# acdha/trivy

Measured on AMD Instinct MI355X. Metric: secret-scan GB/s (builtin rules) at 1/2/4/8 MI355X; % of HBM peak, higher is better.
Workload: dtype u8

## Files before the change

### trivy_amd/csrc/kernels.hip

```cpp
#include <hip/hip_runtime.h>

#include <algorithm>
#include <map>
#include <cstdlib>
#include <cstring>
#include <memory>
#include <vector>

#include "device.hpp"
#include "internal.hpp"
#include "k1f.hpp"

namespace tsg {

#define HIP_TRY(x)                                                                    \
  do {                                                                                \
    hipError_t e_ = (x);                                                              \
    if (e_ != hipSuccess)                                                             \
      return fail(TSG_ERR_GPU, std::string(#x) + ": " + hipGetErrorString(e_));       \
  } while (0)

constexpr int kStreams = 4;
constexpr int kK1Chains = 2;
constexpr int kK1Unroll = 8;
constexpr int kK1Seg = 8;
constexpr int kK1Lds[3] = {52, 80, 156};
constexpr int kK1BlocksPerCU[3] = {3, 2, 1};
constexpr __host__ __device__ int k1_threads(int ldsk) { return ldsk == 156 ? 1024 : 512; }
constexpr uint32_t kK1RepBytes = 256 * 32 * 4;
constexpr int kBlock = 256;
constexpr int kPad = 256;
constexpr int kItemsBpc = 8;
constexpr uint32_t kStampBlocks = 8;
constexpr int kMaxBack = (int)kMaxBackChunks;

struct DevDFA {
  const uint16_t* tab;
  const uint16_t* acc;
  const uint16_t* acc_state;
  const uint16_t* eot;
  const uint16_t* to_ni;
  const uint8_t* dead;
  const uint64_t* masks;
  const uint8_t* cls;
  const uint32_t* rules;
  uint32_t nc, ns, mw, nmasks, state_acc;
  uint32_t nrules;
  uint32_t inv_nc;
  uint32_t start[4];
  uint32_t o_cls, o_dead, o_accs, o_masks, lds_bytes;
};

struct DevK1 {
  const uint16_t* tab;
  const uint32_t* cls;
  const uint32_t* pcls;
  const uint16_t* accs;
  const uint32_t* masks;
  uint32_t nc, ns, nmasks, mw, kw_words, start, warm, kU, kD;
  uint32_t acc_row;
  uint32_t row_unit;
  uint32_t tab_words;
  uint32_t packed;
  uint32_t lds_class;
  uint32_t rep;
  const uint16_t* kw_len;
  uint32_t kw_maxlen;
};

struct DevCand {
  uint32_t file, rule, end;
};

__device__ __forceinline__ uint32_t ctx_of(uint8_t c) {
  if (c == '\n') return 1;
  if ((c >= '0' && c <= '9') || (c >= 'A' && c <= 'Z') || (c >= 'a' && c <= 'z') || c == '_') return 2;
  return 3;
}

__device__ __forceinline__ uint32_t byte_of(const uint4 v, uint32_t k) {
  const uint32_t w = k < 8 ? (k < 4 ? v.x : v.y) : (k < 12 ? v.z : v.w);
  return (w >> ((k & 3) * 8)) & 0xFF;
}

constexpr uint32_t kCfShift = 14;

__device__ __forceinline__ uint32_t bsearch_file(const uint64_t* __restrict__ off, uint32_t lo, uint32_t hi,
                                                 uint64_t p) {
  while (hi - lo > 1) {
    const uint32_t mid = (lo + hi) >> 1;
    if (off[mid] <= p) lo = mid;
    else hi = mid;
  }
  return lo;
}

__device__ __forceinline__ uint32_t file_of(const uint32_t* __restrict__ cf, const uint64_t* __restrict__ off,
                                            uint32_t nfiles, uint64_t p) {
  const uint64_t k = p >> kCfShift;
  return bsearch_file(off, cf[k], min(nfiles, cf[k + 1] + 1), p);
}

__device__ __forceinline__ void stage16(uint8_t* dst, const void* src, uint32_t nbytes) {
// ... 1642 lines not shown
}

__global__ void __launch_bounds__(kBlock) items_emit_kernel(ItemArgs A, LayoutArgs LA) {
  extern __shared__ __attribute__((aligned(16))) uint8_t smem[];
  const ItemLds T = item_lds_load(A, smem);
  uint32_t* s_count = (uint32_t*)(smem + item_lds_bytes(A));
  uint32_t* s_base = s_count + A.G;
  uint32_t* s_gbase = s_base + A.G;
  uint8_t* s_kind = (uint8_t*)(s_gbase + A.G);
  layout_block(LA, s_kind, s_gbase);
  const uint64_t nt = (uint64_t)min(*A.nev, A.evcap) + A.F, stride = (uint64_t)gridDim.x * blockDim.x;
  const uint64_t t0 = (uint64_t)blockIdx.x * blockDim.x + threadIdx.x;
  for (uint32_t g = threadIdx.x; g < A.G; g += blockDim.x) {
    s_base[g] = s_kind[g] == kGroupList ? s_gbase[g] + A.bcount[(size_t)blockIdx.x * A.G + g] : 0u;
    s_count[g] = 0;
  }
  __syncthreads();
  for (uint64_t t = t0; t < nt; t += stride)
    gen_items(A, T, t, [&](uint32_t f, uint32_t g, uint64_t lo, uint64_t hi) {
      if (s_kind[g] != kGroupList) return;
      const uint32_t n = (uint32_t)(hi - lo + 1);
      uint32_t at = s_base[g] + atomicAdd(&s_count[g], n);
      for (uint64_t c = lo; c <= hi; c++) A.items[at++] = make_uint2(f, (uint32_t)c);
    });
}

struct K2Args {
  const uint8_t* data;
  const uint64_t* off;
  const uint32_t* cf;
  uint64_t total, nchunks;
  uint32_t chunk, ext_cap, nfiles;
  const uint32_t* kw;
  uint32_t kw_words;
  const uint32_t* gmask;
  const uint32_t* galways;
  const uint2* items;
  const uint4* entries;
  const uint32_t* nentries;
  const uint4* dentries;
  const uint32_t* ndentries;
  DevCand* cand;
  uint32_t* cand_count;
  uint32_t cand_cap;
  uint8_t* ovf;
  uint8_t* hascand;
  uint32_t* diag;
  uint32_t* claim;
  uint32_t word_recs;
  unsigned long long* etrace;
  unsigned long long* clk;
};
constexpr int kTraceW = 8;
#ifdef K2_TRACE_CTR
__shared__ unsigned long long* s_ectr;
#define K2_CTR(k, op, v) (s_ectr ? (void)op(&s_ectr[k], (unsigned long long)(v)) : (void)0)
#else
#define K2_CTR(k, op, v) ((void)0)
#endif
#ifdef K2_TRACE_PHASE
__shared__ unsigned long long* s_tph;
#define K2_PHASE(k) (s_tph && threadIdx.x == 0 ? (void)(s_tph[k] = wall_clock64()) : (void)0)
#else
#define K2_PHASE(k) ((void)0)
#endif

__device__ __forceinline__ void emit_cand(const K2Args& A, uint32_t file, uint32_t rule, uint64_t end) {
  const unsigned long long m = __ballot(1);
  const uint32_t lane = threadIdx.x & 63;
  const uint32_t leader = (uint32_t)__builtin_ctzll(m);
  uint32_t base = 0;
  if (lane == leader) {
    base = atomicAdd(A.cand_count, (uint32_t)__popcll(m));
    K2_CTR(1, atomicAdd, __popcll(m));
  }
  base = __shfl(base, (int)leader);
  const uint32_t idx = base + (uint32_t)__popcll(m & ((1ull << lane) - 1));
  if (idx < A.cand_cap && (end < kCandWhole || end == (uint64_t)kCandWhole)) {
    A.cand[idx] = DevCand{file, rule, (uint32_t)end};
  } else {
    A.ovf[file] = 1;
    if (idx < A.cand_cap) A.cand[idx] = DevCand{file, rule, 0};
  }
  A.hascand[file] = 1;
}

struct Lane {
  const DevDFA& d;
  const K2Args& A;
  const uint16_t* s_tab;
  const uint8_t* s_cls;
  const uint16_t* s_accs;
  const uint64_t* s_masks;
  uint32_t file;
  uint64_t fs;
  uint32_t group;

  __device__ __forceinline__ void emit(uint32_t mi, uint64_t pos) {
    const uint64_t* m = (d.state_acc && mi < d.nmasks) ? s_masks + (size_t)mi * d.mw : d.masks + (size_t)mi * d.mw;
    for (uint32_t w = 0; w < d.mw; w++)
      for (uint64_t v = m[w]; v; v &= v - 1)
        emit_cand(A, file, d.rules[w * 64 + __builtin_ctzll(v)], pos - fs);
  }

  __device__ __forceinline__ uint32_t state_of(uint32_t row) const { return __umulhi(row, d.inv_nc); }

  __device__ __forceinline__ uint32_t trans(uint32_t ix) const { return kCandTrans | (group << 16) | ix; }
  __device__ __forceinline__ void accept_word(uint32_t s0, const uint4 v, int lo, int hi, uint64_t wb) {
    if (A.word_recs)
      emit_cand(A, file, kCandTrans | kCandWord | (group << 16) | s0, wb + (uint64_t)lo - fs);
    else
      replay_emit(s0, v, lo, hi, wb);
  }
  __device__ __forceinline__ void put(uint32_t idx, uint32_t rule, uint64_t end) const {
    if (idx < A.cand_cap && end < kCandWhole) {
      A.cand[idx] = DevCand{file, rule, (uint32_t)end};
    } else {
      A.ovf[file] = 1;
      if (idx < A.cand_cap) A.cand[idx] = DevCand{file, rule, 0};
    }
    A.hascand[file] = 1;
  }
  __device__ __forceinline__ void replay_emit(uint32_t s0, const uint4 v, int lo, int hi, uint64_t wb) {
    uint32_t n = 0, r = s0;
#pragma unroll
    for (int k = 0; k < 16; k++) {
      const uint32_t e = s_tab[r + s_cls[byte_of(v, k)]];
      const bool in = k >= lo && k < hi;
      n += (in && (e & 0x8000u)) ? 1u : 0u;
      r = in ? (e & 0x7FFFu) : r;
    }
    if (!n) return;
    uint32_t at = atomicAdd(A.cand_count, n);
    K2_CTR(1, atomicAdd, n);
    r = s0;
#pragma unroll
    for (int k = 0; k < 16; k++) {
      const uint32_t ix = r + s_cls[byte_of(v, k)];
      const uint32_t e = s_tab[ix];
      const bool in = k >= lo && k < hi;
      if (in && (e & 0x8000u)) put(at++, trans(ix), wb + k - fs);
      r = in ? (e & 0x7FFFu) : r;
    }
  }

  __device__ __forceinline__ uint32_t step(uint32_t s, uint32_t byte, uint64_t pos) {
    const uint32_t ix = s + s_cls[byte];
    const uint32_t e = s_tab[ix];
    if (__builtin_expect(e & 0x8000u, 0)) emit_cand(A, file, trans(ix), pos - fs);
    return e & 0x7FFFu;
  }

  __device__ __forceinline__ uint32_t fast(uint32_t s, uint32_t byte) const { return s_tab[s + s_cls[byte]]; }

  __device__ __forceinline__ void replay16(uint32_t s, const uint4, uint64_t p) {
#pragma unroll 1
    for (uint32_t k = 0; k < 16; k++) s = step(s, A.data[p + k], p + k);
  }

  __device__ __forceinline__ uint32_t step16(uint32_t s, const uint4 v, uint64_t p) {
    const uint32_t s0 = s;
    uint32_t any = 0;
#pragma unroll
    for (int k = 0; k < 16; k++) {
      const uint32_t e = fast(s, byte_of(v, k));
      any |= e;
      s = e & 0x7FFFu;
    }
    if (__builtin_expect(any & 0x8000u, 0)) replay16(s0, v, p);
    return s;
  }

  __device__ __forceinline__ void tail(uint32_t s, uint64_t fe, uint64_t b) {
    if (b >= fe) {
      const uint32_t m = d.eot[state_of(s)];
      if (m) emit(m, fe);
      return;
    }
    tail_ni(d.to_ni[state_of(s)], fe, b);
  }
  __device__ __forceinline__ void tail_ni(uint32_t s, uint64_t fe, uint64_t b) {
    const uint8_t* data = A.data;
    const uint8_t* dead = s_cls + (d.o_dead - d.o_cls);
    uint64_t q = b;
    uint64_t w = q & ~15ull;
    uint4 cur = *(const uint4*)(data + w);
    while (q < fe && !(dead[state_of(s)] & 1)) {
      if (q - b >= A.ext_cap || (dead[state_of(s)] & 2)) {
        for (uint32_t k = 0; k < d.nrules; k++) emit_cand(A, file, d.rules[k], kCandWhole);
        return;
      }
      const uint4 nxt = *(const uint4*)(data + w + 16);
      const uint64_t e = min(fe, w + 16);
      const int lo = (int)(q - w), hi = (int)(e - w);
      const uint32_t s0 = s;
      uint32_t any = 0;
#pragma unroll
      for (int k = 0; k < 16; k++) {
        const uint32_t t = s_tab[s + s_cls[byte_of(cur, k)]];
        const bool in = k >= lo && k < hi;
        any |= in ? t : 0u;
        s = in ? (t & 0x7FFFu) : s;
      }
      if (__builtin_expect(any & 0x8000u, 0)) accept_word(s0, cur, lo, hi, w);
      q = e;
      cur = nxt;
      w += 16;
    }
    K2_CTR(2, atomicAdd, q - b);
    K2_CTR(3, atomicMax, q - b);
    if (A.diag) {
      const uint32_t n = (uint32_t)min<uint64_t>(q - b, 0xFFFFFFFFull);
      atomicAdd(&A.diag[0], n);
      atomicMax(&A.diag[1], n);
      if (n > 4096) atomicAdd(&A.diag[2], 1u);
    }
    if (q >= fe && !(dead[state_of(s)] & 1)) {
      const uint32_t m = d.eot[state_of(s)];
      if (m) emit(m, fe);
    }
  }

  template <int NS>
  __device__ void streams(uint64_t fe, uint64_t a, uint32_t C) {
    const uint8_t* data = A.data;
    uint32_t s[NS];
#pragma unroll
    for (int i = 0; i < NS; i++) {
      const uint64_t b0 = a + (uint64_t)i * C;
      s[i] = (b0 == fs) ? d.start[0] : d.start[ctx_of(data[b0 - 1])];
    }
    uint4 cur[NS];
#pragma unroll
    for (int i = 0; i < NS; i++) cur[i] = *(const uint4*)(data + a + (uint64_t)i * C);
    for (uint32_t j = 0; j < C; j += 16) {
      uint4 nxt[NS];
#pragma unroll
      for (int i = 0; i < NS; i++) nxt[i] = *(const uint4*)(data + a + (uint64_t)i * C + j + 16);
      uint32_t s0[NS], any[NS];
#pragma unroll
      for (int i = 0; i < NS; i++) {
        s0[i] = s[i];
        any[i] = 0;
      }
#pragma unroll
      for (int k = 0; k < 16; k++)
#pragma unroll
        for (int i = 0; i < NS; i++) {
          const uint32_t e = fast(s[i], byte_of(cur[i], k));
          any[i] |= e;
          s[i] = e & 0x7FFFu;
        }
#pragma unroll
      for (int i = 0; i < NS; i++)
        if (__builtin_expect(any[i] & 0x8000u, 0)) replay16(s0[i], cur[i], a + (uint64_t)i * C + j);
#pragma unroll
      for (int i = 0; i < NS; i++) cur[i] = nxt[i];
    }
#pragma unroll
    for (int i = 0; i < NS; i++) tail(s[i], fe, a + (uint64_t)(i + 1) * C);
  }

  __device__ void piece(uint64_t fe, uint64_t a, uint64_t se) {
    const uint8_t* data = A.data;
    uint32_t s = (a == fs) ? d.start[0] : d.start[ctx_of(data[a - 1])];
    uint64_t p = a;
    while (p < se && (p & 15)) {
      s = step(s, data[p], p);
      p++;
    }
    if (p + 16 <= se) {
      uint4 cur = *(const uint4*)(data + p);
      while (p + 16 <= se) {
        const uint4 nxt = *(const uint4*)(data + p + 16);
        s = step16(s, cur, p);
        cur = nxt;
        p += 16;
      }
    }
    while (p < se) {
      s = step(s, data[p], p);
      p++;
    }
    tail(s, fe, se);
  }
};

__device__ __forceinline__ void stage_dfa(const DevDFA& d, uint8_t* smem) {
  stage16(smem, d.tab, (d.ns * d.nc + 1) / 2 * 4);
  stage16(smem + d.o_cls, d.cls, 256);
  stage16(smem + d.o_dead, d.dead, d.ns);
  if (d.state_acc) {
    stage16(smem + d.o_accs, d.acc_state, d.ns * 2);
    stage16(smem + d.o_masks, d.masks, d.nmasks * d.mw * 8);
  }
  __syncthreads();
}

struct K2Item {
  uint32_t s, file;
  uint32_t lo, hi;
  uint32_t chunk;
  uint64_t fe;
};

template <bool RICH>
__device__ __forceinline__ void k2_list_pair(const DevDFA& d, const K2Args& A, const uint16_t* s_tab,
                                             const uint8_t* s_cls, const uint16_t* s_accs,
                                             const uint64_t* s_masks, uint32_t g, uint32_t first, uint32_t n);

template <bool RICH>
__device__ __forceinline__ void k2_list_entry(const DevDFA& d, const K2Args& A, const uint16_t* s_tab,
                                              const uint8_t* s_cls, const uint16_t* s_accs,
                                              const uint64_t* s_masks, uint4 en) {
  for (uint32_t r0i = 0; r0i < en.z; r0i += 2 * kK2Block)
    k2_list_pair<RICH>(d, A, s_tab, s_cls, s_accs, s_masks, en.x, en.y + r0i, min(en.z - r0i, (uint32_t)(2 * kK2Block)));
}

template <bool RICH>
__device__ __forceinline__ void k2_list_pair(const DevDFA& d, const K2Args& A, const uint16_t* s_tab,
                                             const uint8_t* s_cls, const uint16_t* s_accs,
                                             const uint64_t* s_masks, uint32_t g, uint32_t first, uint32_t n) {
  const uint32_t C = A.chunk;
  K2Item it[2];
  bool live[2];
#pragma unroll
  for (int i = 0; i < 2; i++) {
    const uint32_t k = threadIdx.x + (uint32_t)i * kK2Block;
    live[i] = k < n;
    const uint2 item = A.items[first + (live[i] ? k : 0)];
    it[i].file = item.x;
    it[i].chunk = item.y;
    const uint64_t base = (uint64_t)item.y * C;
    const uint8_t before = base ? A.data[base - 1] : 0;
    const uint64_t fs = A.off[item.x], fe = A.off[item.x + 1];
    const uint64_t a = max(fs, base);
    it[i].fe = fe;
    it[i].lo = (uint32_t)(a - base);
    it[i].hi = live[i] ? (uint32_t)(min(fe, base + C) - base) : it[i].lo;
    it[i].s = a == fs ? d.start[0] : d.start[ctx_of(before)];
  }
  Lane L{d, A, s_tab, s_cls, s_accs, s_masks, 0, 0, g};
  if (C & 127) {
#pragma unroll
    for (int i = 0; i < 2; i++)
      if (live[i]) {
        const uint64_t base = (uint64_t)it[i].chunk * C;
        L.file = it[i].file;
        L.fs = A.off[it[i].file];
        L.piece(A.off[it[i].file + 1], base + it[i].lo, base + it[i].hi);
      }
    return;
  }
  auto word = [&](K2Item& c, uint32_t o, const uint4 v) __attribute__((always_inline)) {
    const int32_t lo = min(16, max(0, (int32_t)c.lo - (int32_t)o));
    const int32_t hi = min(16, max(0, (int32_t)c.hi - (int32_t)o));
    const uint32_t mask = ((1u << hi) - 1u) & ~((1u << lo) - 1u);
    uint32_t s = c.s, any = 0;
    const uint32_t s0 = s;
#pragma unroll
    for (int k = 0; k < 16; k++) {
      const uint32_t e = s_tab[s + s_cls[byte_of(v, k)]];
      const bool in = (mask >> k) & 1u;
      any |= in ? e : 0u;
      s = in ? (e & 0x7FFFu) : s;
    }
    if (__builtin_expect(any & 0x8000u, 0)) {
      if (A.diag) atomicAdd(&A.diag[3], 1u);
      K2_CTR(0, atomicAdd, 1);
      L.file = c.file;
      L.fs = A.off[c.file];
      L.accept_word(s0, v, lo, hi, (uint64_t)c.chunk * C + o);
    }
    c.s = s;
  };
  auto word2 = [&](uint32_t o, const uint4 v0, const uint4 v1) __attribute__((always_inline)) {
    K2Item& c0 = it[0];
    K2Item& c1 = it[1];
    const int32_t lo0 = min(16, max(0, (int32_t)c0.lo - (int32_t)o)), hi0 = min(16, max(0, (int32_t)c0.hi - (int32_t)o));
    const int32_t lo1 = min(16, max(0, (int32_t)c1.lo - (int32_t)o)), hi1 = min(16, max(0, (int32_t)c1.hi - (int32_t)o));
    const uint32_t m0 = ((1u << hi0) - 1u) & ~((1u << lo0) - 1u), m1 = ((1u << hi1) - 1u) & ~((1u << lo1) - 1u);
    uint32_t s0 = c0.s, s1 = c1.s, any0 = 0, any1 = 0;
    const uint32_t r0 = s0, r1 = s1;
#pragma unroll
    for (int k = 0; k < 16; k++) {
      const uint32_t e0 = s_tab[s0 + s_cls[byte_of(v0, k)]];
      const uint32_t e1 = s_tab[s1 + s_cls[byte_of(v1, k)]];
      const bool in0 = (m0 >> k) & 1u, in1 = (m1 >> k) & 1u;
      any0 |= in0 ? e0 : 0u;
      any1 |= in1 ? e1 : 0u;
      s0 = in0 ? (e0 & 0x7FFFu) : s0;
      s1 = in1 ? (e1 & 0x7FFFu) : s1;
    }
    if (__builtin_expect((any0 | any1) & 0x8000u, 0)) {
      if (any0 & 0x8000u) {
        if (A.diag) atomicAdd(&A.diag[3], 1u);
        K2_CTR(0, atomicAdd, 1);
        L.file = c0.file;
        L.fs = A.off[c0.file];
        L.accept_word(r0, v0, lo0, hi0, (uint64_t)c0.chunk * C + o);
      }
      if (any1 & 0x8000u) {
        if (A.diag) atomicAdd(&A.diag[3], 1u);
        K2_CTR(0, atomicAdd, 1);
        L.file = c1.file;
        L.fs = A.off[c1.file];
        L.accept_word(r1, v1, lo1, hi1, (uint64_t)c1.chunk * C + o);
      }
    }
    c0.s = s0;
    c1.s = s1;
  };
  K2_PHASE(1);
  if (__ballot(live[0]) == 0) return;
  const uint32_t lane = threadIdx.x & 63, q = lane & 3;
  const bool b0 = q & 1, b1 = (q >> 1) & 1;
  uint4 x0[4], y0[4];
  const uint8_t* dq = A.data + 16u * q;
#define K2_LOAD_T(X, Y, J, T)                                                                 \
  X[T] = *(const uint4*)(dq + (uint64_t)__shfl(it[0].chunk, (int)((lane & ~3u) + T)) * C + (J)); \
  Y[T] = *(const uint4*)(dq + (uint64_t)__shfl(it[1].chunk, (int)((lane & ~3u) + T)) * C + (J));
#define K2_LOAD(X, Y, J) \
  K2_LOAD_T(X, Y, J, 0)  \
  K2_LOAD_T(X, Y, J, 1)  \
  K2_LOAD_T(X, Y, J, 2)  \
  K2_LOAD_T(X, Y, J, 3)
#define K2_BLOCK(X, Y, J)                                                       \
  quad_transpose4(X, b0, b1);                                                   \
  quad_transpose4(Y, b0, b1);                                                   \
  _Pragma("unroll") for (int w = 0; w < 4; w++) {                              \
    word(it[0], (uint32_t)(J) + 16u * w, X[w]);                                 \
    word(it[1], (uint32_t)(J) + 16u * w, Y[w]);                                 \
  }
  if constexpr (RICH) {
#define K2_BLOCK2(X, Y, J)                                                      \
  quad_transpose4(X, b0, b1);                                                   \
  quad_transpose4(Y, b0, b1);                                                   \
  _Pragma("unroll") for (int w = 0; w < 4; w++) word2((uint32_t)(J) + 16u * w, X[w], Y[w]);
    uint4 x1[4], y1[4];
    K2_LOAD(x0, y0, 0)
    for (uint32_t j = 0; j < C; j += 128) {
      if (j + 64 < C) {
        K2_LOAD(x1, y1, j + 64)
      }
      K2_BLOCK2(x0, y0, j)
      if (j + 64 >= C) break;
      if (j + 128 < C) {
        K2_LOAD(x0, y0, j + 128)
      }
      K2_BLOCK2(x1, y1, j + 64)
    }
#undef K2_BLOCK2
  } else {
    K2_LOAD(x0, y0, 0)
    for (uint32_t j = 0; j < C; j += 64) {
      K2_BLOCK(x0, y0, j)
      if (j + 64 < C) {
        K2_LOAD(x0, y0, j + 64)
      }
    }
  }
#undef K2_LOAD_T
#undef K2_LOAD
#undef K2_BLOCK
  K2_PHASE(2);
  uint32_t ni[2];
#pragma unroll
  for (int i = 0; i < 2; i++) {
    const uint64_t b = (uint64_t)it[i].chunk * C + it[i].hi;
    ni[i] = live[i] && b < it[i].fe ? d.to_ni[L.state_of(it[i].s)] : 0u;
  }
#pragma unroll
  for (int i = 0; i < 2; i++)
    if (live[i]) {
      const uint64_t b = (uint64_t)it[i].chunk * C + it[i].hi;
      L.file = it[i].file;
      L.fs = A.off[it[i].file];
      if (b < it[i].fe)
        L.tail_ni(ni[i], it[i].fe, b);
      else
        L.tail(it[i].s, it[i].fe, b);
    }
  K2_PHASE(3);
}

__device__ __forceinline__ void k2_dense_entry(const DevDFA& d, const K2Args& A, uint32_t g, const uint16_t* s_tab,
                                               const uint8_t* s_cls, const uint16_t* s_accs,
                                               const uint64_t* s_masks, uint4 en) {
  Lane L{d, A, s_tab, s_cls, s_accs, s_masks, 0, 0, g};
  const uint32_t* gm = A.gmask + (size_t)g * A.kw_words;
  const uint32_t always = A.galways[g];
  const uint64_t c0 = en.y + (uint64_t)threadIdx.x * kStreams;
  if (c0 >= (uint64_t)en.y + en.z) return;
  uint64_t a = c0 * A.chunk;
  const uint64_t b = min((c0 + kStreams) * A.chunk, A.total);
  uint32_t f = file_of(A.cf, A.off, A.nfiles, a);
  {
    const uint64_t fs = A.off[f], fe = A.off[f + 1];
    if (b == a + (uint64_t)kStreams * A.chunk && a >= fs && b <= fe) {
      if (group_gated(A.kw + (size_t)f * A.kw_words, gm, A.kw_words, always)) {
        L.file = f;
        L.fs = fs;
        L.template streams<kStreams>(fe, a, A.chunk);
      }
      return;
    }
  }
  while (a < b) {
    const uint64_t fs = A.off[f], fe = A.off[f + 1];
    if (fe <= a) {
      f++;
      continue;
    }
    const uint64_t se = min(b, fe);
    if (group_gated(A.kw + (size_t)f * A.kw_words, gm, A.kw_words, always)) {
      L.file = f;
      L.fs = fs;
      L.piece(fe, a, se);
    }
    a = se;
    f++;
  }
}

template <bool DENSE, bool RICH = false>
__device__ __forceinline__ void k2_run(const DevDFA* __restrict__ dfas, const K2Args& A, const uint4* entries,
                                       uint32_t E, uint32_t* claim, uint8_t* smem) {
  __shared__ uint32_t s_e;
  uint32_t staged = 0xFFFFFFFFu;
  uint32_t prev = 0xFFFFFFFFu;
#ifdef K2_TRACE_CTR
  if (threadIdx.x == 0) s_ectr = nullptr;
#endif
#ifdef K2_TRACE_PHASE
  if (threadIdx.x == 0) s_tph = nullptr;
#endif
  if (E == 0) return;
  bool ran = false;
  for (;;) {
    if (threadIdx.x == 0) s_e = atomicAdd(claim, 1u);
    __syncthreads();
    const uint32_t e = s_e;
    __syncthreads();
    if (!DENSE && A.etrace && threadIdx.x == 0) {
      const unsigned long long now = wall_clock64();
      if (prev != 0xFFFFFFFFu) A.etrace[(size_t)prev * kTraceW + 1] = now;
      if (e < E) {
        const uint4 en = entries[e];
        A.etrace[(size_t)e * kTraceW + 0] = now;
        A.etrace[(size_t)e * kTraceW + 2] = ((unsigned long long)en.x << 32) | en.z;
        A.etrace[(size_t)e * kTraceW + 3] = ((unsigned long long)__builtin_amdgcn_s_getreg(20 | (15 << 11)) << 32) |
                                            (uint32_t)__builtin_amdgcn_s_getreg(4 | (31 << 11));
#ifdef K2_TRACE_CTR
        s_ectr = A.etrace + (size_t)e * kTraceW + 4;
#endif
#ifdef K2_TRACE_PHASE
        s_tph = A.etrace + (size_t)e * kTraceW + 4;
#endif
      }
    }
#if defined(K2_TRACE_CTR) || defined(K2_TRACE_PHASE)
    __syncthreads();
#endif
    prev = e;
    if (e >= E) {
      if (ran && threadIdx.x == 0) atomicMax(&A.clk[kClkK2End], (unsigned long long)wall_clock64());
      break;
    }
    ran = true;
    const uint4 en = entries[e];
    const uint32_t g = __builtin_amdgcn_readfirstlane(en.x);
    const DevDFA& d = dfas[g];
    if (g != staged) {
      stage_dfa(d, smem);
      staged = g;
    }
    K2_PHASE(0);
    const uint16_t* s_tab = (const uint16_t*)smem;
    if (DENSE)
      k2_dense_entry(d, A, g, s_tab, smem + d.o_cls, (const uint16_t*)(smem + d.o_accs), (const uint64_t*)(smem + d.o_masks), en);
    else
      k2_list_entry<RICH>(d, A, s_tab, smem + d.o_cls, (const uint16_t*)(smem + d.o_accs), (const uint64_t*)(smem + d.o_masks), en);
  }
}

__global__ void __launch_bounds__(kK2Block) k2_kernel(const DevDFA* __restrict__ dfas, K2Args A) {
  extern __shared__ __attribute__((aligned(16))) uint8_t smem[];
  k2_run<false>(dfas, A, A.entries, *A.nentries, A.claim, smem);
}
__global__ void __launch_bounds__(kK2Block) __attribute__((amdgpu_waves_per_eu(1, 2)))
k2_kernel_rich(const DevDFA* __restrict__ dfas, K2Args A) {
  extern __shared__ __attribute__((aligned(16))) uint8_t smem[];
  k2_run<false, true>(dfas, A, A.entries, *A.nentries, A.claim, smem);
}

__global__ void __launch_bounds__(kBlock) k2_dense_kernel(const DevDFA* __restrict__ dfas, K2Args A) {
  extern __shared__ __attribute__((aligned(16))) uint8_t smem[];
  k2_run<true>(dfas, A, A.dentries, *A.ndentries, A.claim + 1, smem);
}

template <class T>
static int upload_vec(const std::vector<T>& v, const T** dst, std::vector<void*>* allocs) {
  void* p = nullptr;
  const size_t bytes = (std::max<size_t>(v.size() * sizeof(T), 16) + 15) & ~(size_t)15;
  HIP_TRY(hipMalloc(&p, bytes));
  HIP_TRY(hipMemset(p, 0, bytes));
  if (!v.empty()) HIP_TRY(hipMemcpy(p, v.data(), v.size() * sizeof(T), hipMemcpyHostToDevice));
  allocs->push_back(p);
  *dst = (const T*)p;
  return TSG_OK;
}

static uint32_t align16(uint32_t x) { return (x + 15) & ~15u; }

static int make_device_dfa(const DFA& dd, const std::vector<uint32_t>& rules, DevDFA* out,
                           std::vector<void*>* allocs) {
  if (dd.nstates >= 0x8000) return fail(TSG_ERR_INTERNAL, "DFA too large for u16 tables");
  out->nrules = (uint32_t)rules.size();
  DFA padded;
  const DFA* dp = &dd;
  if (dd.nclasses < 2) {
    padded = dd;
    padded.nclasses = 2;
    padded.next.clear();
    padded.acc.clear();
    for (int st = 0; st < dd.nstates; st++)
      for (int c = 0; c < 2; c++) {
        padded.next.push_back(dd.next[st]);
        padded.acc.push_back(dd.acc[st]);
      }
    dp = &padded;
  }
  const DFA& d = *dp;
  const size_t nc = d.nclasses;
  std::vector<uint16_t> tab((size_t)d.nstates * nc), acc(tab.size()), accs(d.nstates, 0);
  bool state_acc = true;
  if ((size_t)(d.nstates - 1) * nc >= 0x8000) return fail(TSG_ERR_INTERNAL, "DFA rows do not fit 15 bits");
  for (int s = 0; s < d.nstates; s++) {
    uint32_t a0 = d.acc[(size_t)s * nc];
    for (size_t c = 0; c < nc; c++) {
      size_t i = (size_t)s * nc + c;
      if (d.acc[i] > 0xFFFF) return fail(TSG_ERR_INTERNAL, "too many accept masks");
      tab[i] = (uint16_t)((d.next[i] * nc) | (d.acc[i] ? 0x8000u : 0u));
      acc[i] = (uint16_t)d.acc[i];
      if (d.acc[i] != a0) state_acc = false;
    }
    accs[s] = (uint16_t)a0;
  }
  std::vector<uint16_t> eot(d.nstates), ni(d.nstates);
  for (int s = 0; s < d.nstates; s++) {
    eot[s] = (uint16_t)d.eot_acc[s];
    ni[s] = (uint16_t)(d.to_noinject[s] * nc);
  }
  std::vector<uint8_t> dead(d.nstates);
  for (int s = 0; s < d.nstates; s++)
    dead[s] = (d.dead[s] ? 1 : 0) | ((size_t)s < d.immortal.size() && d.immortal[s] ? 2 : 0);
  std::vector<uint64_t> masks;
  for (const auto& m : d.masks) masks.insert(masks.end(), m.begin(), m.end());
  std::vector<uint8_t> cls(d.cls, d.cls + 256);
  std::vector<uint16_t> tabp = tab;
  if (tabp.size() & 1) tabp.push_back(0);
  DevDFA& v = *out;
  int rc;
  if ((rc = upload_vec(tabp, &v.tab, allocs))) return rc;
  if ((rc = upload_vec(acc, &v.acc, allocs))) return rc;
  if ((rc = upload_vec(accs, &v.acc_state, allocs))) return rc;
  if ((rc = upload_vec(eot, &v.eot, allocs))) return rc;
  if ((rc = upload_vec(ni, &v.to_ni, allocs))) return rc;
  if ((rc = upload_vec(dead, &v.dead, allocs))) return rc;
  if ((rc = upload_vec(masks, &v.masks, allocs))) return rc;
  if ((rc = upload_vec(cls, &v.cls, allocs))) return rc;
  if ((rc = upload_vec(rules, &v.rules, allocs))) return rc;
  v.nc = (uint32_t)nc;
  v.ns = (uint32_t)d.nstates;
  v.mw = (uint32_t)d.mask_words;
  v.nmasks = (uint32_t)d.masks.size();
  for (int k = 0; k < 4; k++) v.start[k] = d.start[k] * (uint32_t)nc;
  v.inv_nc = (uint32_t)((0x100000000ull + nc - 1) / nc);
  uint32_t o = align16((uint32_t)(tab.size() * 2));
  v.o_cls = o;
  o += 256;
  v.o_dead = o;
  o += align16((uint32_t)d.nstates);
  v.o_accs = o;
  v.o_masks = o;
  v.state_acc = 0;
  const uint32_t acc_bytes = align16(d.nstates * 2) + align16((uint32_t)masks.size() * 8);
  if (state_acc && o + acc_bytes + 16 * 1024 <= 150 * 1024) {
    v.state_acc = 1;
    v.o_masks = o + align16(d.nstates * 2);
    o += acc_bytes;
  }
  v.lds_bytes = o + 16;
  if (v.lds_bytes > 160 * 1024) return fail(TSG_ERR_INTERNAL, "DFA tables exceed LDS");
  return TSG_OK;
}

struct K1Host {
  std::vector<uint16_t> tab, accs;
  std::vector<uint32_t> masks;
  std::vector<uint32_t> order;
  uint32_t stride = 0;
  uint32_t unit = 1;
};

static int k1_lds_class(size_t tab_bytes) {
  for (int k = 0; k < 3; k++)
    if (tab_bytes + kK1RepBytes <= (size_t)kK1Lds[k] * 1024) return 2 * k + 1;
  return tab_bytes + 1024 <= (size_t)kK1Lds[2] * 1024 ? 2 * 2 : 2 * 3;
}

static bool k1_packed_fits(size_t ns, size_t rs) { return ns * rs * 2 <= 65536; }

static size_t k1_stride(size_t nc, size_t ns) {
  size_t rs = nc;
  while (rs % 4 != 2) rs++;
  auto tab = [&](size_t r) { return (ns * r + (ns * r & 1)) * 2; };
  if (k1_packed_fits(ns, nc)) return k1_packed_fits(ns, rs) ? rs : nc;
  if ((ns - 1) * rs > 0xFFFF || k1_lds_class(tab(rs)) != k1_lds_class(tab(nc))) return nc;
  return rs;
}

static int k1_tables(const Plan& p, const std::vector<uint8_t>& quiet, K1Host* h, uint32_t* start_row,
                     uint32_t* acc_row) {
  const DFA& d = *p.kw_dfa;
  const size_t nc = d.nclasses, ns = d.nstates;
  const size_t rs = k1_stride(nc, ns);
  h->stride = (uint32_t)rs;
  h->unit = k1_packed_fits(ns, rs) ? 2 : 1;
  const size_t row = rs * h->unit;
  if ((ns - 1) * row > 0xFFFF) return fail(TSG_ERR_INTERNAL, "keyword automaton too large for 16-bit rows");
  std::vector<uint32_t> newid(ns);
  h->order.clear();
  for (int pass = 0; pass < 2; pass++)
// ... 558 lines not shown
      HIP_TRY(hipFuncSetAttribute((const void*)items_emit_kernel, hipFuncAttributeMaxDynamicSharedMemorySize, (int)emit_lds));
      HIP_TRY(hipFuncSetAttribute((const void*)items_count_kernel, hipFuncAttributeMaxDynamicSharedMemorySize, (int)emit_lds));
    }
  }
  if (r->max_lds > 64 * 1024) {
    HIP_TRY(hipFuncSetAttribute((const void*)k2_kernel, hipFuncAttributeMaxDynamicSharedMemorySize, (int)r->max_lds));
    HIP_TRY(hipFuncSetAttribute((const void*)k2_kernel_rich, hipFuncAttributeMaxDynamicSharedMemorySize, (int)r->max_lds));
    HIP_TRY(hipFuncSetAttribute((const void*)k2_dense_kernel, hipFuncAttributeMaxDynamicSharedMemorySize,
                                (int)r->max_lds));
  }
  const uint32_t* cg = nullptr;
  if ((rc = upload_vec(gmask, &cg, &r->tables))) return rc;
  r->d_gmask = (uint32_t*)cg;
  if ((rc = upload_vec(galways, &cg, &r->tables))) return rc;
  r->d_galways = (uint32_t*)cg;
  if ((rc = upload_vec(gevents, &cg, &r->tables))) return rc;
  r->d_gevents = (uint32_t*)cg;
  if ((rc = upload_vec(r->gback, &cg, &r->tables))) return rc;
  r->d_gback = (uint32_t*)cg;
  const unsigned long long* cb = nullptr;
  if ((rc = upload_vec(gofbit, &cb, &r->tables))) return rc;
  {
    const uint32_t nkw = (uint32_t)p.kw_words * 32;
    std::vector<unsigned long long> kwg((size_t)nkw * r->GW, 0), galw(r->GW, 0);
    for (uint32_t g = 0; g < G; g++) {
      for (uint32_t k = 0; k < nkw; k++)
        if ((gmask[(size_t)g * p.kw_words + k / 32] >> (k % 32)) & 1) kwg[(size_t)k * r->GW + g / 64] |= 1ull << (g % 64);
      if (galways[g]) galw[g / 64] |= 1ull << (g % 64);
    }
    const unsigned long long* c64 = nullptr;
    if ((rc = upload_vec(kwg, &c64, &r->tables))) return rc;
    r->d_kwg = (unsigned long long*)c64;
    if ((rc = upload_vec(galw, &c64, &r->tables))) return rc;
    r->d_galw = (unsigned long long*)c64;
  }
  r->h_galways = galways;
  r->h_gevents = gevents;
  r->h_gofbit = gofbit;
  r->d_gofbit = (unsigned long long*)cb;
  const DevDFA* cd = nullptr;
  if ((rc = upload_vec(r->groups, &cd, &r->tables))) return rc;
  r->d_groups = (DevDFA*)cd;
  hipDeviceProp_t prop;
  HIP_TRY(hipGetDeviceProperties(&prop, device));
  r->cus = prop.multiProcessorCount;
  r->grid = prop.multiProcessorCount * 8;
  HIP_TRY(hipEventCreateWithFlags(&r->kernels_done, hipEventDisableTiming | hipEventReleaseToDevice));
  int occ = 0;
  HIP_TRY(hipOccupancyMaxActiveBlocksPerMultiprocessor(&occ, (const void*)k2_kernel, kK2Block, r->max_lds));
  r->k2_grid = r->cus * std::max(occ, 1);
  {
    int occ_rich = 0;
    HIP_TRY(hipOccupancyMaxActiveBlocksPerMultiprocessor(&occ_rich, (const void*)k2_kernel_rich, kK2Block, r->max_lds));
    r->k2_rich = occ_rich >= 1 && occ_rich >= occ;
  }
  HIP_TRY(hipOccupancyMaxActiveBlocksPerMultiprocessor(&occ, (const void*)k2_dense_kernel, kBlock, r->max_lds));
  r->k2_dense_grid = r->cus * std::max(occ, 1);
  *out = r.release();
  return TSG_OK;
}

void device_rules_destroy(DeviceRules* d) { delete d; }

std::shared_ptr<const std::vector<uint8_t>> device_rules_kw_unknown(const DeviceRules* d) { return d->kw_unknown; }
uint32_t device_rules_hot_states(const DeviceRules* d) { return d->hot_states; }
bool device_rules_k1_filter(const DeviceRules* d) { return d->use_k1f; }
bool device_rules_k2_rich(const DeviceRules* d) { return d->k2_rich; }

int lane_create(DeviceRules* d, LaneState** out) {
  HIP_TRY(hipSetDevice(d->device));
  auto l = std::make_unique<LaneState>();
  l->d = d;
  HIP_TRY(hipStreamCreateWithFlags(&l->st, hipStreamNonBlocking));
  const uint32_t G = std::max<uint32_t>(1, (uint32_t)d->groups.size());
  HIP_TRY(hipMalloc((void**)&l->counts, sizeof(uint32_t) * kCounts));
  HIP_TRY(hipMalloc((void**)&l->gcount, sizeof(uint32_t) * G));
  HIP_TRY(hipMalloc((void**)&l->bcount, sizeof(uint32_t) * G * (size_t)d->grid));
  HIP_TRY(hipMalloc((void**)&l->cursor, sizeof(uint32_t) * G));
  HIP_TRY(hipMalloc((void**)&l->gskip, G));
  *out = l.release();
  return TSG_OK;
}

void lane_destroy(LaneState* l) { delete l; }
hipStream_t lane_stream(LaneState* l) { return l->st; }

static size_t al256(size_t x) { return (x + 255) & ~(size_t)255; }

void host_out_free(HostOut* o) {
  void* ps[] = {o->blk, o->cand};
  for (void* p : ps)
    if (p) (void)hipHostFree(p);
  for (auto& e : o->ev)
    if (e) (void)hipEventDestroy(e);
  *o = HostOut{};
}

int host_out_alloc(const DeviceRules* d, uint32_t files_cap, uint32_t cand_cap, HostOut* o) {
  HIP_TRY(hipSetDevice(d->device));
  HostOut h;
  h.files_cap = std::max<uint32_t>(files_cap, 1);
  h.cand_cap = std::max<uint32_t>(cand_cap, 1);
  h.groups = std::max<uint32_t>(1, (uint32_t)d->groups.size());
  h.kw_words = (uint32_t)d->plan->kw_words;
  const size_t o_gskip = 256, o_ovf = o_gskip + al256(h.groups), o_kw = o_ovf + al256(h.files_cap),
               bytes = o_kw + al256(sizeof(uint32_t) * (size_t)h.files_cap * h.kw_words);
  auto fail_free = [&](hipError_t e, const char* what) {
// ... 572 lines not shown
```

Before: 56.77.

## Store K2 DFA rows as byte offsets with class table in LDS header

```diff
diff --git a/trivy_amd/csrc/kernels.hip b/trivy_amd/csrc/kernels.hip
--- a/trivy_amd/csrc/kernels.hip
+++ b/trivy_amd/csrc/kernels.hip
@@ -34,6 +34,9 @@
 constexpr uint32_t kStampBlocks = 8;
 constexpr int kMaxBack = (int)kMaxBackChunks;
 
+constexpr uint32_t kK2Tab = 512;
+constexpr uint32_t kK2Acc = 1;
+constexpr uint32_t kK2Row = 0xFFFEu;
 struct DevDFA {
   const uint16_t* tab;
   const uint16_t* acc;
@@ -42,13 +45,13 @@
   const uint16_t* to_ni;
   const uint8_t* dead;
   const uint64_t* masks;
-  const uint8_t* cls;
+  const uint16_t* cls;
   const uint32_t* rules;
   uint32_t nc, ns, mw, nmasks, state_acc;
   uint32_t nrules;
   uint32_t inv_nc;
   uint32_t start[4];
-  uint32_t o_cls, o_dead, o_accs, o_masks, lds_bytes;
+  uint32_t o_dead, o_accs, o_masks, lds_bytes;
 };
 
 struct DevK1 {
@@ -1797,11 +1800,21 @@
   unsigned long long* clk;
 };
 constexpr int kTraceW = 8;
+#if defined(K2_TRACE_CTR) || defined(K2_TRACE_MASK)
+__shared__ unsigned long long* s_ectr;
+#endif
 #ifdef K2_TRACE_CTR
-__shared__ unsigned long long* s_ectr;
 #define K2_CTR(k, op, v) (s_ectr ? (void)op(&s_ectr[k], (unsigned long long)(v)) : (void)0)
 #else
 #define K2_CTR(k, op, v) ((void)0)
+#endif
+#ifdef K2_TRACE_MASK
+#define K2_MASKCTR(masked)                                                                   \
+  ((s_ectr && (threadIdx.x & 63) == 0)                                                       \
+       ? (void)(atomicAdd(&s_ectr[0], 1ull), atomicAdd(&s_ectr[1], (masked) ? 1ull : 0ull)) \
+       : (void)0)
+#else
+#define K2_MASKCTR(masked) ((void)0)
 #endif
 #ifdef K2_TRACE_PHASE
 __shared__ unsigned long long* s_tph;
@@ -1833,8 +1846,8 @@
 struct Lane {
   const DevDFA& d;
   const K2Args& A;
-  const uint16_t* s_tab;
-  const uint8_t* s_cls;
+  const uint8_t* lds;
+  const uint16_t* s_cls;
   const uint16_t* s_accs;
   const uint64_t* s_masks;
   uint32_t file;
@@ -1849,11 +1862,14 @@
   }
 
   __device__ __forceinline__ uint32_t state_of(uint32_t row) const { return __umulhi(row, d.inv_nc); }
-
-  __device__ __forceinline__ uint32_t trans(uint32_t ix) const { return kCandTrans | (group << 16) | ix; }
+  __device__ __forceinline__ uint32_t ent(uint32_t at) const { return *(const uint16_t*)(lds + at); }
+
+  __device__ __forceinline__ uint32_t trans(uint32_t at) const {
+    return kCandTrans | (group << 16) | ((at - kK2Tab) >> 1);
+  }
   __device__ __forceinline__ void accept_word(uint32_t s0, const uint4 v, int lo, int hi, uint64_t wb) {
     if (A.word_recs)
-      emit_cand(A, file, kCandTrans | kCandWord | (group << 16) | s0, wb + (uint64_t)lo - fs);
+      emit_cand(A, file, kCandTrans | kCandWord | (group << 16) | (s0 >> 1), wb + (uint64_t)lo - fs);
     else
       replay_emit(s0, v, lo, hi, wb);
   }
@@ -1870,10 +1886,10 @@
     uint32_t n = 0, r = s0;
 #pragma unroll
     for (int k = 0; k < 16; k++) {
-      const uint32_t e = s_tab[r + s_cls[byte_of(v, k)]];
+      const uint32_t e = ent(r + s_cls[byte_of(v, k)]);
       const bool in = k >= lo && k < hi;
-      n += (in && (e & 0x8000u)) ? 1u : 0u;
-      r = in ? (e & 0x7FFFu) : r;
+      n += (in && (e & kK2Acc)) ? 1u : 0u;
+      r = in ? (e & kK2Row) : r;
     }
     if (!n) return;
     uint32_t at = atomicAdd(A.cand_count, n);
@@ -1882,21 +1898,21 @@
 #pragma unroll
     for (int k = 0; k < 16; k++) {
       const uint32_t ix = r + s_cls[byte_of(v, k)];
-      const uint32_t e = s_tab[ix];
+      const uint32_t e = ent(ix);
       const bool in = k >= lo && k < hi;
-      if (in && (e & 0x8000u)) put(at++, trans(ix), wb + k - fs);
-      r = in ? (e & 0x7FFFu) : r;
+      if (in && (e & kK2Acc)) put(at++, trans(ix), wb + k - fs);
+      r = in ? (e & kK2Row) : r;
     }
   }
 
   __device__ __forceinline__ uint32_t step(uint32_t s, uint32_t byte, uint64_t pos) {
     const uint32_t ix = s + s_cls[byte];
-    const uint32_t e = s_tab[ix];
-    if (__builtin_expect(e & 0x8000u, 0)) emit_cand(A, file, trans(ix), pos - fs);
-    return e & 0x7FFFu;
-  }
-
-  __device__ __forceinline__ uint32_t fast(uint32_t s, uint32_t byte) const { return s_tab[s + s_cls[byte]]; }
+    const uint32_t e = ent(ix);
+    if (__builtin_expect(e & kK2Acc, 0)) emit_cand(A, file, trans(ix), pos - fs);
+    return e & kK2Row;
+  }
+
+  __device__ __forceinline__ uint32_t fast(uint32_t s, uint32_t byte) const { return ent(s + s_cls[byte]); }
 
   __device__ __forceinline__ void replay16(uint32_t s, const uint4, uint64_t p) {
 #pragma unroll 1
@@ -1910,9 +1926,9 @@
     for (int k = 0; k < 16; k++) {
       const uint32_t e = fast(s, byte_of(v, k));
       any |= e;
-      s = e & 0x7FFFu;
-    }
-    if (__builtin_expect(any & 0x8000u, 0)) replay16(s0, v, p);
+      s = e & kK2Row;
+    }
+    if (__builtin_expect(any & kK2Acc, 0)) replay16(s0, v, p);
     return s;
   }
 
@@ -1926,7 +1942,7 @@
   }
   __device__ __forceinline__ void tail_ni(uint32_t s, uint64_t fe, uint64_t b) {
     const uint8_t* data = A.data;
-    const uint8_t* dead = s_cls + (d.o_dead - d.o_cls);
+    const uint8_t* dead = lds + d.o_dead;
     uint64_t q = b;
     uint64_t w = q & ~15ull;
     uint4 cur = *(const uint4*)(data + w);
@@ -1940,14 +1956,23 @@
       const int lo = (int)(q - w), hi = (int)(e - w);
       const uint32_t s0 = s;
       uint32_t any = 0;
-#pragma unroll
-      for (int k = 0; k < 16; k++) {
-        const uint32_t t = s_tab[s + s_cls[byte_of(cur, k)]];
-        const bool in = k >= lo && k < hi;
-        any |= in ? t : 0u;
-        s = in ? (t & 0x7FFFu) : s;
-      }
-      if (__builtin_expect(any & 0x8000u, 0)) accept_word(s0, cur, lo, hi, w);
+      if (lo == 0 && hi == 16) {
+#pragma unroll
+        for (int k = 0; k < 16; k++) {
+          const uint32_t t = fast(s, byte_of(cur, k));
+          any |= t;
+          s = t & kK2Row;
+        }
+      } else {
+#pragma unroll
+        for (int k = 0; k < 16; k++) {
+          const uint32_t t = fast(s, byte_of(cur, k));
+          const bool in = k >= lo && k < hi;
+          any |= in ? t : 0u;
+          s = in ? (t & kK2Row) : s;
+        }
+      }
+      if (__builtin_expect(any & kK2Acc, 0)) accept_word(s0, cur, lo, hi, w);
       q = e;
       cur = nxt;
       w += 16;
@@ -1994,11 +2019,11 @@
         for (int i = 0; i < NS; i++) {
           const uint32_t e = fast(s[i], byte_of(cur[i], k));
           any[i] |= e;
-          s[i] = e & 0x7FFFu;
+          s[i] = e & kK2Row;
         }
 #pragma unroll
       for (int i = 0; i < NS; i++)
-        if (__builtin_expect(any[i] & 0x8000u, 0)) replay16(s0[i], cur[i], a + (uint64_t)i * C + j);
+        if (__builtin_expect(any[i] & kK2Acc, 0)) replay16(s0[i], cur[i], a + (uint64_t)i * C + j);
 #pragma unroll
       for (int i = 0; i < NS; i++) cur[i] = nxt[i];
     }
@@ -2032,8 +2057,8 @@
 };
 
 __device__ __forceinline__ void stage_dfa(const DevDFA& d, uint8_t* smem) {
-  stage16(smem, d.tab, (d.ns * d.nc + 1) / 2 * 4);
-  stage16(smem + d.o_cls, d.cls, 256);
+  stage16(smem, d.cls, kK2Tab);
+  stage16(smem + kK2Tab, d.tab, (d.ns * d.nc + 1) / 2 * 4);
   stage16(smem + d.o_dead, d.dead, d.ns);
   if (d.state_acc) {
     stage16(smem + d.o_accs, d.acc_state, d.ns * 2);
@@ -2050,21 +2075,18 @@
 };
 
 template <bool RICH>
-__device__ __forceinline__ void k2_list_pair(const DevDFA& d, const K2Args& A, const uint16_t* s_tab,
-                                             const uint8_t* s_cls, const uint16_t* s_accs,
+__device__ __forceinline__ void k2_list_pair(const DevDFA& d, const K2Args& A, const uint8_t* lds, const uint16_t* s_accs,
                                              const uint64_t* s_masks, uint32_t g, uint32_t first, uint32_t n);
 
 template <bool RICH>
-__device__ __forceinline__ void k2_list_entry(const DevDFA& d, const K2Args& A, const uint16_t* s_tab,
-                                              const uint8_t* s_cls, const uint16_t* s_accs,
+__device__ __forceinline__ void k2_list_entry(const DevDFA& d, const K2Args& A, const uint8_t* lds, const uint16_t* s_accs,
                                               const uint64_t* s_masks, uint4 en) {
   for (uint32_t r0i = 0; r0i < en.z; r0i += 2 * kK2Block)
-    k2_list_pair<RICH>(d, A, s_tab, s_cls, s_accs, s_masks, en.x, en.y + r0i, min(en.z - r0i, (uint32_t)(2 * kK2Block)));
+    k2_list_pair<RICH>(d, A, lds, s_accs, s_masks, en.x, en.y + r0i, min(en.z - r0i, (uint32_t)(2 * kK2Block)));
 }
 
 template <bool RICH>
-__device__ __forceinline__ void k2_list_pair(const DevDFA& d, const K2Args& A, const uint16_t* s_tab,
-                                             const uint8_t* s_cls, const uint16_t* s_accs,
+__device__ __forceinline__ void k2_list_pair(const DevDFA& d, const K2Args& A, const uint8_t* lds, const uint16_t* s_accs,
                                              const uint64_t* s_masks, uint32_t g, uint32_t first, uint32_t n) {
   const uint32_t C = A.chunk;
   K2Item it[2];
@@ -2085,7 +2107,7 @@
     it[i].hi = live[i] ? (uint32_t)(min(fe, base + C) - base) : it[i].lo;
     it[i].s = a == fs ? d.start[0] : d.start[ctx_of(before)];
   }
-  Lane L{d, A, s_tab, s_cls, s_accs, s_masks, 0, 0, g};
+  Lane L{d, A, lds, (const uint16_t*)lds, s_accs, s_masks, 0, 0, g};
   if (C & 127) {
 #pragma unroll
     for (int i = 0; i < 2; i++)
@@ -2097,60 +2119,94 @@
       }
     return;
   }
-  auto word = [&](K2Item& c, uint32_t o, const uint4 v) __attribute__((always_inline)) {
-    const int32_t lo = min(16, max(0, (int32_t)c.lo - (int32_t)o));
-    const int32_t hi = min(16, max(0, (int32_t)c.hi - (int32_t)o));
-    const uint32_t mask = ((1u << hi) - 1u) & ~((1u << lo) - 1u);
+  auto clamp16 = [](uint32_t x, uint32_t o) __attribute__((always_inline)) {
+    return min(16, max(0, (int32_t)x - (int32_t)o));
+  };
+  auto inside = [&](int i, uint32_t o) __attribute__((always_inline)) {
+    return !live[i] || (it[i].lo <= o && it[i].hi >= o + 16u);
+  };
+  auto word = [&](int i, uint32_t o, const uint4 v) __attribute__((always_inline)) {
+    K2Item& c = it[i];
     uint32_t s = c.s, any = 0;
     const uint32_t s0 = s;
-#pragma unroll
-    for (int k = 0; k < 16; k++) {
-      const uint32_t e = s_tab[s + s_cls[byte_of(v, k)]];
-      const bool in = (mask >> k) & 1u;
-      any |= in ? e : 0u;
-      s = in ? (e & 0x7FFFu) : s;
-    }
-    if (__builtin_expect(any & 0x8000u, 0)) {
+    const bool whole = __ballot(!inside(i, o)) == 0;
+    K2_MASKCTR(!whole);
+    if (whole) {
+#pragma unroll
+      for (int k = 0; k < 16; k++) {
+        const uint32_t e = L.fast(s, byte_of(v, k));
+        any |= e;
+        s = e & kK2Row;
+      }
+      any = live[i] ? any : 0u;
+    } else {
+      const int32_t lo = clamp16(c.lo, o), hi = clamp16(c.hi, o);
+      const uint32_t mask = ((1u << hi) - 1u) & ~((1u << lo) - 1u);
+#pragma unroll
+      for (int k = 0; k < 16; k++) {
+        const uint32_t e = L.fast(s, byte_of(v, k));
+        const bool in = (mask >> k) & 1u;
+        any |= in ? e : 0u;
+        s = in ? (e & kK2Row) : s;
+      }
+    }
+    if (__builtin_expect(any & kK2Acc, 0)) {
       if (A.diag) atomicAdd(&A.diag[3], 1u);
       K2_CTR(0, atomicAdd, 1);
       L.file = c.file;
       L.fs = A.off[c.file];
-      L.accept_word(s0, v, lo, hi, (uint64_t)c.chunk * C + o);
+      L.accept_word(s0, v, clamp16(c.lo, o), clamp16(c.hi, o), (uint64_t)c.chunk * C + o);
     }
     c.s = s;
   };
   auto word2 = [&](uint32_t o, const uint4 v0, const uint4 v1) __attribute__((always_inline)) {
     K2Item& c0 = it[0];
     K2Item& c1 = it[1];
-    const int32_t lo0 = min(16, max(0, (int32_t)c0.lo - (int32_t)o)), hi0 = min(16, max(0, (int32_t)c0.hi - (int32_t)o));
-    const int32_t lo1 = min(16, max(0, (int32_t)c1.lo - (int32_t)o)), hi1 = min(16, max(0, (int32_t)c1.hi - (int32_t)o));
-    const uint32_t m0 = ((1u << hi0) - 1u) & ~((1u << lo0) - 1u), m1 = ((1u << hi1) - 1u) & ~((1u << lo1) - 1u);
     uint32_t s0 = c0.s, s1 = c1.s, any0 = 0, any1 = 0;
     const uint32_t r0 = s0, r1 = s1;
-#pragma unroll
-    for (int k = 0; k < 16; k++) {
-      const uint32_t e0 = s_tab[s0 + s_cls[byte_of(v0, k)]];
-      const uint32_t e1 = s_tab[s1 + s_cls[byte_of(v1, k)]];
-      const bool in0 = (m0 >> k) & 1u, in1 = (m1 >> k) & 1u;
-      any0 |= in0 ? e0 : 0u;
-      any1 |= in1 ? e1 : 0u;
-      s0 = in0 ? (e0 & 0x7FFFu) : s0;
-      s1 = in1 ? (e1 & 0x7FFFu) : s1;
-    }
-    if (__builtin_expect((any0 | any1) & 0x8000u, 0)) {
-      if (any0 & 0x8000u) {
+    const bool whole = __ballot(!(inside(0, o) && inside(1, o))) == 0;
+    K2_MASKCTR(!whole);
+    if (whole) {
+#pragma unroll
+      for (int k = 0; k < 16; k++) {
+        const uint32_t e0 = L.fast(s0, byte_of(v0, k));
+        const uint32_t e1 = L.fast(s1, byte_of(v1, k));
+        any0 |= e0;
+        any1 |= e1;
+        s0 = e0 & kK2Row;
+        s1 = e1 & kK2Row;
+      }
+      any0 = live[0] ? any0 : 0u;
+      any1 = live[1] ? any1 : 0u;
+    } else {
+      const int32_t lo0 = clamp16(c0.lo, o), hi0 = clamp16(c0.hi, o);
+      const int32_t lo1 = clamp16(c1.lo, o), hi1 = clamp16(c1.hi, o);
+      const uint32_t m0 = ((1u << hi0) - 1u) & ~((1u << lo0) - 1u), m1 = ((1u << hi1) - 1u) & ~((1u << lo1) - 1u);
+#pragma unroll
+      for (int k = 0; k < 16; k++) {
+        const uint32_t e0 = L.fast(s0, byte_of(v0, k));
+        const uint32_t e1 = L.fast(s1, byte_of(v1, k));
+        const bool in0 = (m0 >> k) & 1u, in1 = (m1 >> k) & 1u;
+        any0 |= in0 ? e0 : 0u;
+        any1 |= in1 ? e1 : 0u;
+        s0 = in0 ? (e0 & kK2Row) : s0;
+        s1 = in1 ? (e1 & kK2Row) : s1;
+      }
+    }
+    if (__builtin_expect((any0 | any1) & kK2Acc, 0)) {
+      if (any0 & kK2Acc) {
         if (A.diag) atomicAdd(&A.diag[3], 1u);
         K2_CTR(0, atomicAdd, 1);
         L.file = c0.file;
         L.fs = A.off[c0.file];
-        L.accept_word(r0, v0, lo0, hi0, (uint64_t)c0.chunk * C + o);
-      }
-      if (any1 & 0x8000u) {
+        L.accept_word(r0, v0, clamp16(c0.lo, o), clamp16(c0.hi, o), (uint64_t)c0.chunk * C + o);
+      }
+      if (any1 & kK2Acc) {
         if (A.diag) atomicAdd(&A.diag[3], 1u);
         K2_CTR(0, atomicAdd, 1);
         L.file = c1.file;
         L.fs = A.off[c1.file];
-        L.accept_word(r1, v1, lo1, hi1, (uint64_t)c1.chunk * C + o);
+        L.accept_word(r1, v1, clamp16(c1.lo, o), clamp16(c1.hi, o), (uint64_t)c1.chunk * C + o);
       }
     }
     c0.s = s0;
@@ -2174,8 +2230,8 @@
   quad_transpose4(X, b0, b1);                                                   \
   quad_transpose4(Y, b0, b1);                                                   \
   _Pragma("unroll") for (int w = 0; w < 4; w++) {                              \
-    word(it[0], (uint32_t)(J) + 16u * w, X[w]);                                 \
-    word(it[1], (uint32_t)(J) + 16u * w, Y[w]);                                 \
+    word(0, (uint32_t)(J) + 16u * w, X[w]);                                     \
+    word(1, (uint32_t)(J) + 16u * w, Y[w]);                                     \
   }
   if constexpr (RICH) {
 #define K2_BLOCK2(X, Y, J)                                                      \
@@ -2229,10 +2285,9 @@
   K2_PHASE(3);
 }
 
-__device__ __forceinline__ void k2_dense_entry(const DevDFA& d, const K2Args& A, uint32_t g, const uint16_t* s_tab,
-                                               const uint8_t* s_cls, const uint16_t* s_accs,
+__device__ __forceinline__ void k2_dense_entry(const DevDFA& d, const K2Args& A, uint32_t g, const uint8_t* lds, const uint16_t* s_accs,
                                                const uint64_t* s_masks, uint4 en) {
-  Lane L{d, A, s_tab, s_cls, s_accs, s_masks, 0, 0, g};
+  Lane L{d, A, lds, (const uint16_t*)lds, s_accs, s_masks, 0, 0, g};
   const uint32_t* gm = A.gmask + (size_t)g * A.kw_words;
   const uint32_t always = A.galways[g];
   const uint64_t c0 = en.y + (uint64_t)threadIdx.x * kStreams;
@@ -2274,7 +2329,7 @@
   __shared__ uint32_t s_e;
   uint32_t staged = 0xFFFFFFFFu;
   uint32_t prev = 0xFFFFFFFFu;
-#ifdef K2_TRACE_CTR
+#if defined(K2_TRACE_CTR) || defined(K2_TRACE_MASK)
   if (threadIdx.x == 0) s_ectr = nullptr;
 #endif
 #ifdef K2_TRACE_PHASE
@@ -2296,7 +2351,7 @@
         A.etrace[(size_t)e * kTraceW + 2] = ((unsigned long long)en.x << 32) | en.z;
         A.etrace[(size_t)e * kTraceW + 3] = ((unsigned long long)__builtin_amdgcn_s_getreg(20 | (15 << 11)) << 32) |
                                             (uint32_t)__builtin_amdgcn_s_getreg(4 | (31 << 11));
-#ifdef K2_TRACE_CTR
+#if defined(K2_TRACE_CTR) || defined(K2_TRACE_MASK)
         s_ectr = A.etrace + (size_t)e * kTraceW + 4;
 #endif
 #ifdef K2_TRACE_PHASE
@@ -2304,7 +2359,7 @@
 #endif
       }
     }
-#if defined(K2_TRACE_CTR) || defined(K2_TRACE_PHASE)
+#if defined(K2_TRACE_CTR) || defined(K2_TRACE_PHASE) || defined(K2_TRACE_MASK)
     __syncthreads();
 #endif
     prev = e;
@@ -2321,11 +2376,10 @@
       staged = g;
     }
     K2_PHASE(0);
-    const uint16_t* s_tab = (const uint16_t*)smem;
     if (DENSE)
-      k2_dense_entry(d, A, g, s_tab, smem + d.o_cls, (const uint16_t*)(smem + d.o_accs), (const uint64_t*)(smem + d.o_masks), en);
+      k2_dense_entry(d, A, g, smem, (const uint16_t*)(smem + d.o_accs), (const uint64_t*)(smem + d.o_masks), en);
     else
-      k2_list_entry<RICH>(d, A, s_tab, smem + d.o_cls, (const uint16_t*)(smem + d.o_accs), (const uint64_t*)(smem + d.o_masks), en);
+      k2_list_entry<RICH>(d, A, smem, (const uint16_t*)(smem + d.o_accs), (const uint64_t*)(smem + d.o_masks), en);
   }
 }
 
@@ -2381,12 +2435,13 @@
   std::vector<uint16_t> tab((size_t)d.nstates * nc), acc(tab.size()), accs(d.nstates, 0);
   bool state_acc = true;
   if ((size_t)(d.nstates - 1) * nc >= 0x8000) return fail(TSG_ERR_INTERNAL, "DFA rows do not fit 15 bits");
+  if (nc > 256) return fail(TSG_ERR_INTERNAL, "DFA has more than 256 classes");
   for (int s = 0; s < d.nstates; s++) {
     uint32_t a0 = d.acc[(size_t)s * nc];
     for (size_t c = 0; c < nc; c++) {
       size_t i = (size_t)s * nc + c;
       if (d.acc[i] > 0xFFFF) return fail(TSG_ERR_INTERNAL, "too many accept masks");
-      tab[i] = (uint16_t)((d.next[i] * nc) | (d.acc[i] ? 0x8000u : 0u));
+      tab[i] = (uint16_t)((d.next[i] * nc * 2) | (d.acc[i] ? kK2Acc : 0u));
       acc[i] = (uint16_t)d.acc[i];
       if (d.acc[i] != a0) state_acc = false;
     }
@@ -2395,14 +2450,15 @@
   std::vector<uint16_t> eot(d.nstates), ni(d.nstates);
   for (int s = 0; s < d.nstates; s++) {
     eot[s] = (uint16_t)d.eot_acc[s];
-    ni[s] = (uint16_t)(d.to_noinject[s] * nc);
+    ni[s] = (uint16_t)(d.to_noinject[s] * nc * 2);
   }
   std::vector<uint8_t> dead(d.nstates);
   for (int s = 0; s < d.nstates; s++)
     dead[s] = (d.dead[s] ? 1 : 0) | ((size_t)s < d.immortal.size() && d.immortal[s] ? 2 : 0);
   std::vector<uint64_t> masks;
   for (const auto& m : d.masks) masks.insert(masks.end(), m.begin(), m.end());
-  std::vector<uint8_t> cls(d.cls, d.cls + 256);
+  std::vector<uint16_t> cls(256);
+  for (int b = 0; b < 256; b++) cls[b] = (uint16_t)(d.cls[b] * 2 + kK2Tab);
   std::vector<uint16_t> tabp = tab;
   if (tabp.size() & 1) tabp.push_back(0);
   DevDFA& v = *out;
@@ -2420,11 +2476,9 @@
   v.ns = (uint32_t)d.nstates;
   v.mw = (uint32_t)d.mask_words;
   v.nmasks = (uint32_t)d.masks.size();
-  for (int k = 0; k < 4; k++) v.start[k] = d.start[k] * (uint32_t)nc;
-  v.inv_nc = (uint32_t)((0x100000000ull + nc - 1) / nc);
-  uint32_t o = align16((uint32_t)(tab.size() * 2));
-  v.o_cls = o;
-  o += 256;
+  for (int k = 0; k < 4; k++) v.start[k] = d.start[k] * (uint32_t)nc * 2;
+  v.inv_nc = (uint32_t)((0x100000000ull + 2 * nc - 1) / (2 * nc));
+  uint32_t o = kK2Tab + align16((uint32_t)(tab.size() * 2));
   v.o_dead = o;
   o += align16((uint32_t)d.nstates);
   v.o_accs = o;
@@ -3089,7 +3143,7 @@
   {
     int occ_rich = 0;
     HIP_TRY(hipOccupancyMaxActiveBlocksPerMultiprocessor(&occ_rich, (const void*)k2_kernel_rich, kK2Block, r->max_lds));
-    r->k2_rich = occ_rich >= 1 && occ_rich >= occ;
+    r->k2_rich = occ_rich >= 1 && std::min(occ_rich, 2) >= occ;
   }
   HIP_TRY(hipOccupancyMaxActiveBlocksPerMultiprocessor(&occ, (const void*)k2_dense_kernel, kBlock, r->max_lds));
   r->k2_dense_grid = r->cus * std::max(occ, 1);
```

Measured after the change: 56.72. About the same (-0.1%).
